# mit-acl/clipper

Measured on AMD Instinct MI355X. Metric: affinity+solve ms and GEMV HBM GB/s, n=10k assoc, 95% outliers, 1/8 GPU, lower is better.
Workload: dtype f64 (M stored f32)

## Files before the change

### clipper_amd/csrc/host_solver.hpp

```cpp
#pragma once

namespace {

using Ctx = clipper_hip_ctx;

void rowview_free(Shard& s);
void rowview_drop(Ctx* h);
void sub_free(Ctx* h);

int free_shard_buffers(Shard& s) {
  hipSetDevice(s.device);
  auto fr = [](auto*& p) {
    if (p) hipFree(p);
    p = nullptr;
  };
  fr(s.S);
  fr(s.Cs);
  fr(s.part);
  fr(s.u0);
  fr(s.pt);
  fr(s.cab);
  fr(s.X[0]);
  fr(s.X[1]);
  fr(s.ab);
// ... 83 lines not shown
  for (auto& s : h->sh) {
    free_shard_buffers(s);
    HIPCHK(hipSetDevice(s.device));
    const size_t bytesS = static_cast<size_t>(m) * static_cast<size_t>(W) * h->esize();
    s.bytes_S = bytesS;
    if (!h->compressed) HIPCHK(hipMalloc(&s.S, bytesS));
    const size_t nvec = static_cast<size_t>(P * W) * sizeof(double);
    const size_t V = static_cast<size_t>(h->V);
    HIPCHK(hipMalloc(&s.u0, nvec));
    const size_t NSLOT = static_cast<size_t>(nslot(h->V));
    HIPCHK(hipMalloc(&s.pt, 2 * V * 2 * nvec));
    HIPCHK(hipMalloc(&s.cab, 2 * nvec));
    for (int k = 0; k < 2; ++k) {
      HIPCHK(hipMalloc(&s.X[k], (V + 1) * VS * nvec));
      HIPCHK(hipMemsetAsync(s.X[k], 0, (V + 1) * VS * nvec, s.stream));
    }
    const size_t Q = static_cast<size_t>(tail_q(h->V));
    const size_t nwg = static_cast<size_t>(ceil_div(m, TAIL_THREADS));
    HIPCHK(hipMalloc(&s.scal, (nwg + ceil_div(nwg, SCAL_FOLD) + 1) * Q * sizeof(double)));
    HIPCHK(hipMalloc(&s.ab, NSLOT * nvec));
    HIPCHK(hipMemsetAsync(s.ab, 0, NSLOT * nvec, s.stream));
    s.part_tiles = static_cast<size_t>(max_tiles(h));
    HIPCHK(hipMalloc(&s.part, s.part_tiles * NSLOT * W * sizeof(double)));
    HIPCHK(hipMalloc(&s.st, 2 * sizeof(SolverState)));
    HIPCHK(hipMemsetAsync(s.st, 0, 2 * sizeof(SolverState), s.stream));
    HIPCHK(hipMalloc(&s.shared, sizeof(SolveShared)));
    HIPCHK(hipMalloc(&s.marks, KIND_CAP));
    HIPCHK(hipMemsetAsync(s.marks, 0, KIND_CAP, s.stream));
    HIPCHK(hipMemsetAsync(s.shared, 0, sizeof(SolveShared), s.stream));
  }
  h->alloc_m = m;
  h->alloc_W = W;
  h->has_matrix = false;
  h->csc_valid = false;
  h->explicitC = false;
  plan_tiles(h);
  h->u0_staged = false;
  h->staged_d = 0;
  return 0;
}

template <typename T, bool HASC, int V>
void launch_pass_tv(Ctx* h, Shard& s, const SolveArgs& a) {
  constexpr int UNR = gemv_unr(V, sizeof(T), HASC);
  dim3 grid(h->nstrips, h->ntiles), block(GEMV_NW * 64);
  hipLaunchKernelGGL((k_gemv<T, HASC, V, GEMV_NW, UNR>), grid, block, 0, s.stream,
                     static_cast<const T*>(s.S), static_cast<const T*>(s.Cs), h->rows_per_tile, a);
}
// ... 120 lines not shown
  for (auto& q : h->sh) {
    HIPCHK(hipSetDevice(q.device));
    for (auto& p : h->sh) {
      if (p.slot == q.slot) continue;
      HIPCHK(hipStreamWaitEvent(q.stream, p.ev_reduced, 0));
      const int64_t off = static_cast<int64_t>(p.slot) * blk_elems;
      if (p.device == q.device) {
        HIPCHK(hipMemcpyAsync(q.ab + off, p.ab + off, blk, hipMemcpyDeviceToDevice, q.stream));
      } else {
        HIPCHK(hipMemcpyPeerAsync(q.ab + off, q.device, p.ab + off, p.device, blk, q.stream));
      }
    }
    HIPCHK(hipEventRecord(q.ev_copied, q.stream));
  }
  for (auto& p : h->sh) {
    HIPCHK(hipSetDevice(p.device));
    for (auto& q : h->sh) {
      if (p.slot == q.slot) continue;
      HIPCHK(hipStreamWaitEvent(p.stream, q.ev_copied, 0));
    }
  }
  return 0;
}

SolveArgs solve_args(Ctx* h, Shard& s, const SolverParams& prm, int par, bool decide_only) {
  SolveArgs a;
  a.st_cur = s.st + par;
  a.st_next = s.st + (par ^ 1);
  a.shared = s.shared;
  a.host = (&s == &h->sh[0]) ? h->mirror_dev : nullptr;
  a.prm = prm;
  a.m = h->m;
  a.W = h->W;
  a.mp = h->mp;
  a.u0 = s.u0;
  a.pt = s.pt;
  a.cab = s.cab;
  a.Xin = s.X[par];
  a.Xout = s.X[par ^ 1];
  a.ab = s.ab;
  a.part = s.part;
  a.ntiles = h->csc_valid ? s.s_nslots : h->ntiles;
  a.slot = s.slot;
  a.scal = s.scal;
  a.nwg = static_cast<int>(ceil_div(h->m, TAIL_THREADS));
  a.scal_in = s.scal;
// ... 16 lines not shown
  a.rvp = h->rvp;
  a.decide_only = decide_only ? 1 : 0;
  a.adaptive_window = (h->csc_valid && h->world == 1 && !h->multiproc && h->sh.size() == 1 && h->adaptive_window) ? 1 : 0;
  a.sub_state = 0;
  a.sub_ncol = 0.0;
  a.colmap = nullptr;
  if (h->parent != nullptr) {
    Ctx* p = h->parent;
    a.host = p->mirror_dev;
    a.host_u = p->u_pinned_dev;
    a.marks = p->profiling ? p->sh[0].marks : nullptr;
    a.kind = a.marks ? p->kind_dev : nullptr;
    a.stamps = p->stamps_dev;
    a.stamps_wide = p->stamps_rows > 4096 ? 1 : 0;
    a.sub_state = 2;
    a.sub_ncol = p->sub.ncol;
    a.colmap = p->sub.colmap;
    static const int test_leave = std::getenv("CLIPPER_HIP_SUB_TEST_LEAVE") ? std::atoi(std::getenv("CLIPPER_HIP_SUB_TEST_LEAVE")) : 0;
    if (test_leave > 0 && p->sub.launches_since_entry >= test_leave) a.sub_ncol = 1e300;
  } else if (h->sub.ready && !h->sub.active && !decide_only) {
    a.sub_state = 1;
    a.sub_ncol = h->sub.ncol;
  }
  return a;
}

template <int V>
int enqueue_iteration_v(Ctx* h, const SolverParams& prm, bool decide_only) {
  const int par = h->par;
  h->par ^= 1;
  const bool sharded = !(h->world == 1 && !h->multiproc);
  Shard& s0 = h->sh[0];
  constexpr int every = PROFILE_EVERY;
  Ctx* hp = h->parent != nullptr ? h->parent : h;
  const bool prof = hp->profiling && (hp->launch_counter % every == 4 || hp->launch_counter == 11) &&
                    hp->ev_used < MAX_EVENT_PAIRS;
  for (auto& s : h->sh) {
    HIPCHK(hipSetDevice(s.device));
    const SolveArgs a = solve_args(h, s, prm, par, decide_only);
    if (prof && &s == &s0) HIPCHK(hipEventRecord(hp->ev_pairs[2 * hp->ev_used], s.stream));
    if (h->csc_valid) launch_pass_csc<V>(h, s, a);
    else launch_pass<V>(h, s, a);
    if (prof && &s == &s0) {
      HIPCHK(hipEventRecord(hp->ev_pairs[2 * hp->ev_used + 1], s.stream));
      hp->ev_launch_index[hp->ev_used] = hp->launch_counter;
      ++hp->ev_used;
// ... 177 lines not shown
    return nullptr;
  }
  std::memset(h->mirror, 0, sizeof(HostMirror));
  if (hipHostMalloc(reinterpret_cast<void**>(&h->kind), KIND_CAP,
                    hipHostMallocMapped | hipHostMallocCoherent) != hipSuccess ||
      hipHostGetDevicePointer(reinterpret_cast<void**>(&h->kind_dev), h->kind, 0) != hipSuccess) {
    fail(CLIPPER_HIP_E_HIP, "cannot allocate the pinned iteration marks");
    destroy_ctx(h);
    return nullptr;
  }
  std::memset(h->kind, 0, KIND_CAP);
  if (const char* e = std::getenv("CLIPPER_HIP_STAMPS")) {
    h->stamps_rows = std::atoi(e) == 2 ? 16384 : 4096;
    const size_t bytes = static_cast<size_t>(h->stamps_rows) * 4 * sizeof(long long);
    if (hipMalloc(&h->stamps_dev, bytes) == hipSuccess) (void)hipMemset(h->stamps_dev, 0, bytes);
    else h->stamps_dev = nullptr;
  }
  if (const char* w = std::getenv("CLIPPER_HIP_WINDOW")) {
    const int v = std::atoi(w);
    if (v == 1 || v == 4 || v == 6 || v == 8) h->V_forced = v;
  }
  if (const char* e = std::getenv("CLIPPER_HIP_ADAPTIVE_WINDOW"))
    if (std::atoi(e) == 0) h->adaptive_window = false;
  if (const char* e = std::getenv("CLIPPER_HIP_RESIDENT"))
    if (std::atoi(e) == 0) h->resident_mode = 1;
  return h;
}

template <typename T>
int ensure_cap(T*& p, size_t& cap, size_t bytes) {
  if (bytes <= cap && p) return 0;
  if (p) hipFree(p);
  p = nullptr;
  cap = 0;
  HIPCHK(hipMalloc(&p, bytes));
  cap = bytes;
  return 0;
}

int upload_points(Ctx* h, Shard& s, const double* D1, const double* D2, int d, int64_t n1,
                  int64_t n2, int64_t pstride, const StagedInputs* dev = nullptr) {
  const size_t b1 = static_cast<size_t>(d) * n1 * sizeof(double);
  const size_t b2 = static_cast<size_t>(d) * n2 * sizeof(double);
  const size_t bp = static_cast<size_t>(d) * pstride * sizeof(double);
  const size_t ba = static_cast<size_t>(2 * h->m) * sizeof(int32_t);
  int rc;
// ... 126 lines not shown
```

### clipper_amd/csrc/host_state.hpp

```cpp
#pragma once

namespace {

thread_local std::string g_err;

int fail(int code, const char* fmt, ...) {
  char buf[512];
  va_list ap;
  va_start(ap, fmt);
  vsnprintf(buf, sizeof(buf), fmt, ap);
  va_end(ap);
  g_err = buf;
  return code;
}

int guard_fail(int code, const char* what) noexcept {
  try {
    g_err = what;
  } catch (...) {
  }
  return code;
}
#define CLIPPER_HIP_GUARD_CATCH(on_nomem, on_other)                                                     \
  catch (const std::bad_alloc&) { on_nomem; }                                                            \
// ... 289 lines not shown
  const SolverParams* solve_prm = nullptr;
  bool early_decide_done = false;
  int resident_mode = 0;
  bool borrowed_stream = false;
  int last_solver = 0;

  int fill_kind = 0;
  EuclidParams fill_e{};
  PointNormalParams fill_n{};
  float fill_E2 = 0.f;
  double total_slice_bytes = 0.0;
  ViewPolicy rvp{};
  bool rv_fresh = false;
  int rv_mode = 0;
  SliceView* rv_desc_host = nullptr;
  int rv_desc_slot = 0;
  SliceView* rv_desc_host_dev = nullptr;
  int32_t* rv_count = nullptr;
  int32_t* rv_count_dev = nullptr;
  clipper_hip_view_stats_t rv_stats{};
  SubProblem sub;
  struct clipper_hip_ctx* parent = nullptr;
  bool adaptive_window = true;
  int sub_mode = 0;

  long long* stamps_dev = nullptr;
  int stamps_rows = 4096;
  bool profiling = false;
  int profiling_level = 0;
  std::vector<hipEvent_t> ev_pairs;
  std::vector<int64_t> ev_launch_index;
  std::vector<hipEvent_t> ev_xchg;
  std::vector<char> ev_xchg_used;
  int ev_used = 0;
  int64_t launch_counter = 0;
  clipper_hip_timings_t tm{};

  size_t esize() const { return storage == CLIPPER_HIP_STORE_F64 ? 8 : 4; }
};
```

### clipper_amd/csrc/host_subproblem.hpp

```cpp
#pragma once

namespace {

bool sub_enabled(const Ctx* h) {
  static const bool env_off = [] {
    const char* e = std::getenv("CLIPPER_HIP_SUBPROBLEM");
    return e && std::atoi(e) == 0;
  }();
  static const int64_t min_m = std::getenv("CLIPPER_HIP_SUBPROBLEM_MIN_M") ? std::atoll(std::getenv("CLIPPER_HIP_SUBPROBLEM_MIN_M")) : SUB_MIN_M;
  return !env_off && h->sub_mode != 1 && h->parent == nullptr && h->sh.size() == 1 && h->world == 1 && !h->multiproc &&
         h->csc_valid && !h->explicitC && h->m >= min_m && rect_fill_possible(h);
}

void sub_begin_solve(Ctx* h) {
  SubProblem& sp = h->sub;
  sp.ready = sp.active = false;
  sp.entries = 0;
  sp.sub_passes = sp.leaves = 0;
  sp.build_ms = 0.0;
}

void sub_free(Ctx* h) {
  SubProblem& sp = h->sub;
  for (Ctx** pc : {&sp.ctx, &sp.ctx_dense}) {
// ... 149 lines not shown
                 (c->csc_valid ? static_cast<double>(c->sh[0].s_bytes) : algorithmic_gemv_bytes(c)) * 1e-6, sp.build_ms);
  return 0;
}

int sub_prepare(Ctx* h) {
  int rc = 0;
  dispatch_window(h, [&](auto v) { rc = sub_prepare_v<decltype(v)::value>(h); });
  return rc;
}

int sub_enter(Ctx* h, const SolverParams& prm) {
  SubProblem& sp = h->sub;
  if (!sp.ready || sp.active || !sp.use) return fail(CLIPPER_HIP_E_INTERNAL, "sub-problem: a hand-over nobody prepared");
  Shard& s = h->sh[0];
  Ctx* c = sp.use;
  Shard& cs = c->sh[0];
  HIPCHK(hipSetDevice(s.device));
  hipLaunchKernelGGL(k_sub_resume, dim3(1), dim3(64), 0, s.stream, s.st + h->par, s.shared);
  if (int rc = enqueue_iteration(h, prm, true)) return rc;
  std::memset(h->u_pinned, 0, static_cast<size_t>(h->m) * sizeof(double));
  std::atomic_thread_fence(std::memory_order_seq_cst);
  hipLaunchKernelGGL(k_sub_enter, dim3(static_cast<unsigned>(ceil_div(c->mp, 256))), dim3(256), 0, s.stream, s.st + h->par, s.pt,
                     s.cab, h->mp, h->V, sp.colmap, sp.nS, cs.st, cs.shared, cs.pt, cs.cab, c->mp,
                     c->csc_valid ? static_cast<double*>(nullptr) : cs.X[0], prm.beta);
  c->par = 0;
  c->rv_fresh = false;
  sp.active = true;
  sp.entries += 1;
  sp.launches_since_entry = 0;
  sp.passes_at_entry = h->mirror->n_passes;
  h->rv_stats.sub_entries += 1;
  return 0;
}

int sub_leave(Ctx* h) {
  SubProblem& sp = h->sub;
  if (!sp.active || !sp.use) return fail(CLIPPER_HIP_E_INTERNAL, "sub-problem: nothing to leave");
  Shard& s = h->sh[0];
  Ctx* c = sp.use;
  Shard& cs = c->sh[0];
  HIPCHK(hipSetDevice(s.device));
  hipLaunchKernelGGL(k_sub_leave, dim3(static_cast<unsigned>(ceil_div(h->mp, 256))), dim3(256), 0, s.stream, cs.st + c->par, cs.pt,
                     cs.cab, c->mp, h->V, sp.pos, s.rv.in_view[s.rv.cur], h->m, s.pt, s.cab, h->mp, sp.nout_acc);
  hipLaunchKernelGGL(k_sub_leave_state, dim3(1), dim3(256), 0, s.stream, cs.st + c->par, s.st + h->par, s.shared, sp.nout_acc);
  sp.active = false;
  sp.leaves += 1;
  if (sp.entries >= SUB_MAX_ENTRIES) sp.ready = false;
// ... 5 lines not shown
```

### clipper_amd/csrc/k_solver.hip.h

```cpp
#pragma once

#include <hip/hip_runtime.h>
#include <stdint.h>
#include <type_traits>


namespace clipper_hip {


constexpr int VS = 8;
constexpr int nslot(int V) { return V + 1; }
constexpr int tail_nr(int V) { return 3 + 2 * V; }
constexpr int tail_q(int V) { return V * tail_nr(V) + 2 * V + 2; }

constexpr double LIVE_OUT = 67108864.0;
constexpr double RV_GAIN_MARGIN = 1.3;
constexpr double RV_ROWS_RATIO = 0.8;

struct ViewPolicy {
  int32_t on;
  int32_t max_builds;
  double pass_fixed, pass_per_row;
  double build_fixed, build_per_row;
};
// ... 21 lines not shown
  double sx[VS];
  int32_t sel;
  int32_t ubp, ubv;
  int32_t phase;
  int32_t stage;
  int32_t i, j, k;
  int64_t n_passes;
  int64_t n_trials;
  int64_t n_iters;
  int32_t nlive;
  int32_t nout;
  int32_t view;
  int32_t hold;
  int64_t n_view_passes;
  int32_t rv_builds;
  int32_t rv_last;
  int32_t rv_backoff;
  int32_t hold_slot;
  int32_t hold_nlive;
  int32_t resume;
  int32_t weff;
  int32_t zero_run;
  int32_t n_redo;
  int32_t pad_;
};

struct SolveShared {
  double F, d;
  int64_t n_passes, n_trials;
  int32_t ifinal, ubp, ubv;
  int32_t done;
  int32_t hold;
  int32_t pad;
};

struct HostMirror {
  double F, d;
  int64_t n_passes, n_trials;
  int64_t iters;
  int32_t ifinal, ubp, ubv;
  int32_t done;
  int32_t nlive, nout;
  int64_t n_view_passes;
  int32_t hold;
  int32_t hold_nlive;
};

// ... 4 lines not shown
  double tol_u, tol_F, beta, eps;
  int32_t maxiniters, maxoliters, maxlsiters;
};


__device__ __forceinline__ double cl_project(double u, double al, double g) {
  const double t = u + al * g;
  return (t > 0.0) ? t : 0.0;
}

__device__ __forceinline__ double cl_norm(double z, bool use = true) { return (use && z > 0.0) ? sqrt(z) : 1.0; }

__device__ __forceinline__ double cl_grad(double d, double x, double s, double a, double b) {
  return (1 + d) * x - d * s + a + b * d;
}
__device__ __forceinline__ double cl_grad_fused(double d, double x, double s, double gs) {
  return (1 + d) * x - d * s + gs;
}

__device__ __forceinline__ double cl_pen_cbu(double s, double b, double u) { return s - b - u; }
__device__ __forceinline__ bool cl_pen_in(double cbu, double u, double eps) { return cbu > eps && u > eps; }
__device__ __forceinline__ double cl_pen_ratio(double a, double u, double cbu) { return fabs((a + u) / cbu); }
__device__ __forceinline__ double cl_pen_ratio_init(double a, double u, double cbu) { return (a + u) / cbu; }

constexpr double SUB_ENTER_MARGIN = 1.10;
constexpr double SUB_STAY_MARGIN = 1.01;

constexpr int TAIL_THREADS = 256;
constexpr int TAIL_WAVES = TAIL_THREADS / 64;
constexpr int TAIL_SPLIT = 1;

struct SolveArgs {
  const SolverState* st_cur;
  SolverState* st_next;
  SolveShared* shared;
  HostMirror* host;
  SolverParams prm;
  int64_t m;
  int64_t W;
  int64_t mp;
  const double* u0;
  double* pt;
  double* cab;
  const double* Xin;
  double* Xout;
  double* ab;
  double* part;
  int ntiles;
  int slot;
  double* scal;
  int nwg;
  const double* scal_in;
  int nwg_in;
  uint8_t* marks;
  uint8_t* kind;
  double* host_u;
  long long* stamps;
  int stamps_wide;
  const uint8_t* in_view;
  int rv_nslots;
  int rv_nwork;
  int rv_fresh;
  int rv_rows;
  ViewPolicy rvp;
  int decide_only;
  int adaptive_window;
  int sub_state;
  double sub_ncol;
  const int32_t* colmap;
};
constexpr int KIND_CAP = 1 << 16;


__device__ __forceinline__ double* pt_arr(const SolveArgs& A, int V, int p, int v, int k) {
  return A.pt + ((static_cast<int64_t>(p) * V + v) * 2 + k) * A.mp;
}

template <int CTRL, int ROW_MASK>
__device__ __forceinline__ double dpp_f64(double v) {
  const int lo = __builtin_amdgcn_update_dpp(0, __double2loint(v), CTRL, ROW_MASK, 0xf, false);
  const int hi = __builtin_amdgcn_update_dpp(0, __double2hiint(v), CTRL, ROW_MASK, 0xf, false);
  return __hiloint2double(hi, lo);
}

__device__ __forceinline__ double wave_sum_to_lane63(double v) {
  v += dpp_f64<0xB1, 0xf>(v);
  v += dpp_f64<0x4E, 0xf>(v);
  v += dpp_f64<0x141, 0xf>(v);
  v += dpp_f64<0x140, 0xf>(v);
  v += dpp_f64<0x142, 0xa>(v);
  v += dpp_f64<0x143, 0xc>(v);
  return v;
// ... 196 lines not shown
  int i_ = L.i, j_ = L.j, k_ = L.k, ubp = L.ubp, ubv = L.ubv, sel = L.sel;
  const int wprev = (L.weff >= 1 && L.weff <= V) ? L.weff : V;
  int zero_run = L.zero_run;
  int64_t n_passes = L.n_passes, n_trials = L.n_trials;
  const int64_t n_iters = L.n_iters + 1;
  int nlive = L.nlive, nout = L.nout;
  auto live_code = [&](double code) {
    const double o = floor(code * (1.0 / LIVE_OUT));
    nout = static_cast<int>(o);
    nlive = static_cast<int>(code - o * LIVE_OUT);
  };
  if (writer && tid == 0) {
#pragma unroll
    for (int l = 0; l < V; ++l) {
      stash->nrm[l] = 1.0;
      stash->sx[l] = 0.0;
    }
  }
  enum { ACT_PASS, ACT_BUILD, ACT_SLOW, ACT_DONE };
  int action = ACT_SLOW;
  int next_phase = PH_TRIAL;
  bool need_pair = false;
  bool redo = false;
  bool sub_ok = true;
  auto sub_bound = [&](const double* sums, int nb) {
    if (A.sub_state == 0) return;
    const double kap = (A.sub_state == 1 ? SUB_ENTER_MARGIN : SUB_STAY_MARGIN) * A.sub_ncol;
    const double lhs = d * d, rhs = (1.0 + d) * (1.0 + d) * kap;
#pragma unroll
    for (int l = 0; l < V; ++l) {
      const double z = sums[nb + 2 * l], sl = sums[nb + 2 * l + 1];
      sub_ok = sub_ok && (lhs * sl * sl >= rhs * z);
    }
  };

  if (phase == PH_TRIAL || phase == PH_BUILD) {
    {
      red[tid] = L.chain;
      __syncthreads();
      double tot = 0.0;
      if (tid < QPAD) {
        tot = red[tid];
#pragma unroll
        for (int c2 = 1; c2 < NCH; ++c2) tot += red[c2 * QPAD + tid];
      }
      __syncthreads();
// ... 103 lines not shown
      } else {
        alpha = 1.0;
        k_ = 0;
        sel = 0;
        action = ACT_PASS;
        sub_bound(sums, 2);
        if (writer && tid == 0) {
#pragma unroll
          for (int l = 0; l < V; ++l) {
            const double nl = cl_norm(sums[2 + 2 * l]);
            stash->nrm[l] = nl;
            stash->sx[l] = sums[3 + 2 * l] / nl;
          }
        }
      }
    }
  }

  if (action == ACT_SLOW) {
    if (!writer) return false;
    nlive = nout = static_cast<int>(m < 0x7fffffff ? m : 0x7fffffff);
    const double* ca_ = A.cab;
    const double* cb_ = A.cab + A.mp;
    if (phase == PH_NORMALIZE || phase == PH_RESCALE) {
      double* u = pt_arr(A, V, ubp, ubv, 0);
      double z[1] = {0.0};
      VEC_CHUNKS(base) {
        double uv[VU], av[VU];
        VEC_EACH(k, i, base) {
          uv[k] = A.u0[i];
          if (phase == PH_RESCALE) av[k] = ca_[i];
        }
        VEC_EACH(k, i, base) {
          const double ui = (phase == PH_RESCALE) ? av[k] + uv[k] : uv[k];
          u[i] = ui;
          z[0] += ui * ui;
        }
      }
      block_reduce<1, NWV>(z, scratch);
      const double n0 = sqrt(z[0]);
      VEC_CHUNKS(base) {
        double uv[VU];
        VEC_EACH(k, i, base) uv[k] = u[i];
        VEC_EACH(k, i, base) {
          const double ui = uv[k] / n0;
          u[i] = ui;
          const double row[VS] = {ui, 0.0, 0.0, 0.0, 0.0, 0.0, 0.0, 0.0};
          store_row(A.Xout + i * VS, row);
        }
      }
      sel = 0;
      next_phase = PH_INIT;
    } else {
      if (phase == PH_INIT) {
        const double* u = pt_arr(A, V, ubp, ubv, 0);
        double sv[1] = {0.0};
        VEC_CHUNKS(base) {
          double uv[VU];
          VEC_EACH(k, i, base) uv[k] = u[i];
          VEC_EACH(k, i, base) sv[0] += uv[k];
        }
        block_reduce<1, NWV>(sv, scratch);
        s = sv[0];
        double ca[2] = {0.0, 0.0};
        VEC_CHUNKS(base) {
          double uv[VU], av[VU], bv[VU];
          VEC_EACH(k, i, base) {
            uv[k] = u[i];
            av[k] = ca_[i];
            bv[k] = cb_[i];
          }
          VEC_EACH(k, i, base) {
            const double cbu = cl_pen_cbu(s, bv[k], uv[k]);
            if (cl_pen_in(cbu, uv[k], P.eps)) {
              ca[0] += 1.0;
              ca[1] += cl_pen_ratio_init(av[k], uv[k], cbu);
            }
          }
        }
        block_reduce<2, NWV>(ca, scratch);
        d = (ca[0] > 0.0) ? ca[1] / ca[0] : 0.0;
        i_ = 0;
        action = (i_ >= P.maxoliters) ? ACT_DONE : ACT_BUILD;
      } else {
        const double* u = pt_arr(A, V, ubp, ubv, 0);
        double ca[2] = {0.0, 0.0};
        VEC_CHUNKS(base) {
          double uv[VU], av[VU], bv[VU];
          VEC_EACH(k, i, base) {
            uv[k] = u[i];
            av[k] = ca_[i];
            bv[k] = cb_[i];
          }
          VEC_EACH(k, i, base) {
            const double cbu = cl_pen_cbu(s, bv[k], uv[k]);
            if (cl_pen_in(cbu, uv[k], P.eps)) {
              ca[0] += 1.0;
              ca[1] += cl_pen_ratio(av[k], uv[k], cbu);
            }
          }
        }
        block_reduce<2, NWV>(ca, scratch);
        if (ca[0] > 0.0) {
          d += ca[1] / ca[0];
          ++i_;
          action = (i_ >= P.maxoliters) ? ACT_DONE : ACT_BUILD;
        } else {
          action = ACT_DONE;
        }
      }
    }
  }

  if (writer && action == ACT_DONE && A.host_u != nullptr) {
    const double* u = pt_arr(A, V, ubp, ubv, 0);
    for (int64_t i = tid; i < m; i += NT)
      __hip_atomic_store(A.host_u + (A.colmap != nullptr ? static_cast<int64_t>(A.colmap[i]) : i), u[i], __ATOMIC_RELAXED,
                         __HIP_MEMORY_SCOPE_SYSTEM);
    if (A.kind != nullptr && A.marks != nullptr) {
      const int64_t n = (n_iters < KIND_CAP) ? n_iters : KIND_CAP;
      for (int64_t i = tid; i < n; i += NT)
        __hip_atomic_store(A.kind + i, A.marks[i], __ATOMIC_RELAXED, __HIP_MEMORY_SCOPE_SYSTEM);
    }
    __threadfence_system();
    __syncthreads();
  }

  if (A.rv_fresh != 0 && action != ACT_SLOW) nout = 0;
  auto put_on_hold = [&](int reason) {
    if (writer) {
      copy_state(A.st_next, st, tid, NT);
      __syncthreads();
// ... 40 lines not shown
      o->ubv = ubv;
      o->phase = (action == ACT_BUILD) ? static_cast<int>(PH_BUILD) : next_phase;
      o->stage = (action == ACT_SLOW) ? ST_PASS : ST_RESULTS;
      o->i = i_;
      o->j = j_;
      o->k = k_;
      o->n_passes = n_passes + (action == ACT_PASS ? 1 : 0);
      o->n_trials = n_trials;
      o->n_iters = n_iters;
      o->nlive = nlive;
      o->nout = nout;
      o->view = (action == ACT_PASS && on_view) ? 1 : 0;
      o->hold = 0;
      o->n_view_passes = L.n_view_passes + ((action == ACT_PASS && on_view) ? 1 : 0);
      o->rv_builds = L.rv_builds;
      o->rv_last = L.rv_last;
      o->rv_backoff = L.rv_backoff;
      o->hold_slot = 0;
      o->hold_nlive = 0;
      o->resume = 0;
      o->weff = wnext;
      o->zero_run = zero_run;
      o->n_redo = L.n_redo + (redo ? 1 : 0);
      o->pad_ = 0;
    };
    if (action == ACT_PASS) record(stash, true);
    else record(A.st_next, false);
    if ((A.decide_only != 0 || sub_leave) && action == ACT_PASS) {
      stash->stage = ST_PASS;
      stash->resume = need_pair ? 2 : 1;
      stash->n_passes = n_passes;
      stash->view = 0;
      stash->n_view_passes = L.n_view_passes;
      if (sub_leave) {
        stash->hold = HOLD_SUB_LEAVE;
        A.shared->hold = HOLD_SUB_LEAVE;
      }
    }
    if (action == ACT_DONE) {
      SolveShared* sh = A.shared;
      sh->F = F;
      sh->d = d;
      sh->n_passes = n_passes;
      sh->n_trials = n_trials;
      sh->ifinal = i_;
      sh->ubp = ubp;
      sh->ubv = ubv;
// ... 92 lines not shown
            al = al * beta;
          }
        }
      }
      block_reduce<2 * V, NT / 64>(r, lds);
      if (threadIdx.x == 0) {
#pragma unroll
        for (int l = 0; l < V; ++l) {
          const double z = (all_rows ? 0.0 : stash->nrm[l]) + r[2 * l], sm = (all_rows ? 0.0 : stash->sx[l]) + r[2 * l + 1];
          const double nl = cl_norm(z);
          stash->nrm[l] = nl;
          stash->sx[l] = sm / nl;
        }
      }
      __syncthreads();
    }
    if (threadIdx.x == 0) {
      stash->stage = ST_RESULTS;
      stash->n_passes = L.n_passes + 1;
      stash->n_iters = L.n_iters + 1;
      stash->view = on_view;
      stash->n_view_passes = L.n_view_passes + on_view;
      stash->resume = 0;
      stash->weff = plan.weff;
    }
  }
  return true;
}

__device__ __forceinline__ void flush_state(const SolveArgs& A, const SolverState* stash) {
  if (!is_writer_block()) return;
  copy_state(A.st_next, stash, threadIdx.x, blockDim.x);
  if (threadIdx.x == 0) {
    const int64_t n_iters = stash->n_iters;
    if (A.marks != nullptr && n_iters <= KIND_CAP)
      A.marks[n_iters - 1] = A.sub_state == 2 ? (stash->phase == PH_TRIAL ? MARK_SUB_WINDOW : MARK_SUB_PAIR)
                             : stash->view   ? MARK_VIEW
                                             : (stash->phase == PH_TRIAL ? MARK_WINDOW : MARK_PAIR);
    if (A.host != nullptr) {
      __hip_atomic_store(&A.host->nlive, stash->nlive, __ATOMIC_RELAXED, __HIP_MEMORY_SCOPE_SYSTEM);
      __hip_atomic_store(&A.host->nout, stash->nout, __ATOMIC_RELAXED, __HIP_MEMORY_SCOPE_SYSTEM);
      __hip_atomic_store(&A.host->n_view_passes, stash->n_view_passes, __ATOMIC_RELAXED, __HIP_MEMORY_SCOPE_SYSTEM);
      __hip_atomic_store(&A.host->n_passes, stash->n_passes, __ATOMIC_RELAXED, __HIP_MEMORY_SCOPE_SYSTEM);
      __hip_atomic_store(&A.host->iters, n_iters, __ATOMIC_RELEASE, __HIP_MEMORY_SCOPE_SYSTEM);
    }
  }
}

__global__ __launch_bounds__(256) void k_init(SolveArgs A, SolverState init, SolverState* st0,
                                               double* X0) {
  const int64_t i = static_cast<int64_t>(blockIdx.x) * 256 + threadIdx.x;
  if (i < A.m) {
    const double row[VS] = {A.u0[i], 0.0, 0.0, 0.0, 0.0, 0.0, 0.0, 0.0};
    store_row(X0 + i * VS, row);
  }
  if (blockIdx.x == 0) {
    if (threadIdx.x == 0) {
      *st0 = init;
      A.shared->done = 0;
      A.shared->hold = 0;
    }
  }
}

constexpr int SCAL_FOLD = 32;
constexpr int SCAL_FOLD_MIN = 64;
__global__ __launch_bounds__(128) void k_scal_fold(const double* __restrict__ scal, int nwg, int Q,
                                                    double* __restrict__ out,
                                                    const SolveShared* __restrict__ shared) {
  if (shared->done) return;
  const int w0 = blockIdx.x * SCAL_FOLD;
  const int w1 = (w0 + SCAL_FOLD < nwg) ? w0 + SCAL_FOLD : nwg;
  for (int q = threadIdx.x; q < Q; q += 128) {
    double x[SCAL_FOLD];
#pragma unroll
    for (int k = 0; k < SCAL_FOLD; ++k) {
      const int w = (w0 + k < w1) ? w0 + k : w1 - 1;
      x[k] = scal[static_cast<int64_t>(w) * Q + q];
    }
    double acc = 0.0;
#pragma unroll
    for (int k = 0; k < SCAL_FOLD; ++k)
      if (w0 + k < w1) acc += x[k];
    out[static_cast<int64_t>(blockIdx.x) * Q + q] = acc;
  }
}

template <int V, bool FUSED_REDUCE, bool TABLES = true>
__global__ __launch_bounds__(TAIL_THREADS * (FUSED_REDUCE ? TAIL_SPLIT : 1)) void k_tail(SolveArgs A) {
  constexpr int NR = tail_nr(V);
  constexpr int Q = tail_q(V);
  constexpr int NRED = NR + 2 * V + 2;
  constexpr int NSLOT = nslot(V);
  constexpr int NTW = TAIL_WAVES * (FUSED_REDUCE ? TAIL_SPLIT : 1);
  __shared__ double red[NTW * NRED > 2 * TAIL_SPLIT * TAIL_THREADS ? NTW * NRED : 2 * TAIL_SPLIT * TAIL_THREADS];
  const int v = blockIdx.y;
  const long long c0 = A.stamps ? wall_clock64() : 0;
  const SolverState* st = A.st_next;
  const int te = threadIdx.x & (TAIL_THREADS - 1);
  const int grp = threadIdx.x / TAIL_THREADS;
  const int64_t i = static_cast<int64_t>(blockIdx.x) * TAIL_THREADS + te;
  const bool valid = i < A.m && grp == 0;
  const int done = A.shared->done;
  const int stage = st->stage, phase = st->phase;
  const int ubp = st->ubp, ubv = st->ubv, sel = st->sel;
  const double d = st->d, alpha = st->alpha, s_cur = st->s;
  const double nrmv = st->nrm[v], sxv = st->sx[v];
  const int weff = (st->weff >= 1 && st->weff <= V) ? st->weff : V;
  const int nslots_pass = st->view ? A.rv_nslots : A.ntiles;
  const double live_w = (valid && A.in_view != nullptr && A.in_view[i] == 0) ? 1.0 + LIVE_OUT : 1.0;

  double p0 = 0.0, p1 = 0.0;
  if (FUSED_REDUCE) {
    const int64_t o1 = (v == 0) ? static_cast<int64_t>(V) * A.W : 0;
    const int per = (nslots_pass + TAIL_SPLIT - 1) / TAIL_SPLIT;
    const int t0 = grp * per, t1 = (t0 + per < nslots_pass) ? t0 + per : nslots_pass;
    if (i < A.m) {
      const double* p = A.part + static_cast<int64_t>(v) * A.W + i;
      const int64_t ts = static_cast<int64_t>(NSLOT) * A.W;
      for (int t = t0; t < t1; t += 16) {
        double va[16], vb[16];
#pragma unroll
        for (int q = 0; q < 16; ++q) {
          const int tt = (t + q < t1) ? t + q : t1 - 1;
          va[q] = p[static_cast<int64_t>(tt) * ts];
          vb[q] = p[static_cast<int64_t>(tt) * ts + o1];
        }
#pragma unroll
        for (int q = 0; q < 16; ++q) {
          if (t + q < t1) {
// ... 6 lines not shown
    if constexpr (TAIL_SPLIT > 1) {
      red[(grp * 2 + 0) * TAIL_THREADS + te] = p0;
      red[(grp * 2 + 1) * TAIL_THREADS + te] = p1;
      __syncthreads();
      p0 = red[te];
      p1 = red[TAIL_THREADS + te];
#pragma unroll
      for (int g = 1; g < TAIL_SPLIT; ++g) {
        p0 += red[(g * 2 + 0) * TAIL_THREADS + te];
        p1 += red[(g * 2 + 1) * TAIL_THREADS + te];
      }
      __syncthreads();
    }
  } else if (valid) {
    const int64_t o1 = (v == 0) ? static_cast<int64_t>(V) * A.W : 0;
    const uint32_t pb = static_cast<uint32_t>(i) / static_cast<uint32_t>(A.W);
    const int64_t off = i - static_cast<int64_t>(pb) * A.W;
    const double* blk = A.ab + (static_cast<int64_t>(pb) * NSLOT) * A.W;
    p0 = blk[static_cast<int64_t>(v) * A.W + off];
    p1 = blk[o1 + off];
  }
  if (done) return;
  if (st->hold) return;
  if (stage != ST_RESULTS) return;
  if (phase == PH_TRIAL && v >= weff) return;
  const long long c1 = A.stamps ? wall_clock64() + (p0 > 1e300 ? 1 : 0) : 0;

  if (phase != PH_TRIAL && phase != PH_BUILD) {
    if (v == 0 && valid) {
      A.cab[i] = p0;
      A.cab[A.mp + i] = p1;
    }
    return;
  }
  const double beta = A.prm.beta;
  double r[NRED];
#pragma unroll
  for (int q = 0; q < NRED; ++q) r[q] = 0.0;

  if (phase == PH_BUILD) {
    if (v != 0) return;
    if (valid) {
      const double ui = pt_arr(A, V, ubp, ubv, 0)[i];
      const double gi = (1 + d) * ui - d * s_cur + A.cab[i] + A.cab[A.mp + i] * d;
      pt_arr(A, V, ubp, ubv, 1)[i] = gi;
      r[0] = ui * gi;
      r[NR - 1] = (ui > 0.0 || gi > 0.0) ? live_w : 0.0;
      double row[VS] = {0.0, 0.0, 0.0, 0.0, 0.0, 0.0, 0.0, 0.0};
      double al = 1.0;
#pragma unroll
      for (int l = 0; l < V; ++l) {
        const double t = cl_project(ui, al, gi);
        row[l] = t;
        r[2 + 2 * l] = t * t;
        r[3 + 2 * l] = t;
// ... 84 lines not shown
```

### clipper_amd/csrc/k_subproblem.hip.h

```cpp
#pragma once

#include <hip/hip_runtime.h>
#include <stdint.h>

#include "k_rowview.hip.h"
#include "k_slices.hip.h"
#include "k_solver.hip.h"

namespace clipper_hip {

constexpr double SUB_THETA = 0.4;

__global__ __launch_bounds__(256) void k_sub_colcount(SliceView RV, int32_t* __restrict__ cnt, int64_t mp) {
  const int lane = threadIdx.x & 63;
  const int cg = blockIdx.x * 4 + (threadIdx.x >> 6);
  if (cg >= RV.ncg) return;
  const uint64_t* pre = RV.Pre + static_cast<int64_t>(cg) * RV.nchunks;
  int tot = 0;
  for (int k0 = 0; k0 < RV.nchunks; k0 += 8) {
    uint8_t nq[8];
#pragma unroll
    for (int j = 0; j < 8; ++j) {
      const int k = (k0 + j < RV.nchunks) ? k0 + j : RV.nchunks - 1;
      nq[j] = RV.data[16 * pre[k] + 16 + lane];
// ... 77 lines not shown
}

__global__ __launch_bounds__(256) void k_sub_gather_points(const double* __restrict__ P, const float* __restrict__ Pf,
                                                            int d, int64_t pstride, const int32_t* __restrict__ A,
                                                            int64_t m, const int32_t* __restrict__ colmap, int64_t nS,
                                                            int64_t qstride, double* __restrict__ Q,
                                                            float* __restrict__ Qf, int32_t* __restrict__ B,
                                                            int which) {
  const int64_t i = static_cast<int64_t>(blockIdx.x) * 256 + threadIdx.x;
  if (i >= qstride) return;
  const int64_t c = (i < nS) ? colmap[i] : 0;
  for (int k = 0; k < d; ++k) {
    Q[k * qstride + i] = (i < nS) ? P[k * pstride + c] : 0.0;
    Qf[k * qstride + i] = (i < nS) ? Pf[k * pstride + c] : 0.f;
  }
  if (i < nS) B[which * nS + i] = A[which * m + c];
}

__global__ __launch_bounds__(256) void k_sub_enter(const SolverState* __restrict__ pst, const double* __restrict__ ppt,
                                                    const double* __restrict__ pcab, int64_t pmp, int V,
                                                    const int32_t* __restrict__ colmap, int64_t nS,
                                                    SolverState* __restrict__ cst, SolveShared* __restrict__ cshared,
                                                    double* __restrict__ cpt, double* __restrict__ ccab, int64_t cmp,
                                                    double* __restrict__ ctab, double beta) {
  const int64_t i = static_cast<int64_t>(blockIdx.x) * 256 + threadIdx.x;
  const int64_t slot = static_cast<int64_t>(pst->ubp) * V + pst->ubv;
  if (i < cmp) {
    const bool in = i < nS;
    const int64_t c = in ? colmap[i] : 0;
    const double ui = in ? ppt[(slot * 2 + 0) * pmp + c] : 0.0;
    const double gi = in ? ppt[(slot * 2 + 1) * pmp + c] : 0.0;
    cpt[(slot * 2 + 0) * cmp + i] = ui;
    cpt[(slot * 2 + 1) * cmp + i] = gi;
    ccab[i] = in ? pcab[c] : 0.0;
    ccab[cmp + i] = in ? pcab[pmp + c] : 0.0;
    if (ctab != nullptr && pst->resume == 1) {
      double row[VS] = {0.0, 0.0, 0.0, 0.0, 0.0, 0.0, 0.0, 0.0};
      double al = pst->alpha;
      for (int l = 0; l < V; ++l) {
        row[l] = cl_project(ui, al, gi);
        al = al * beta;
      }
      store_row(ctab + (static_cast<int64_t>(pst->sel) * cmp + i) * VS, row);
    }
  }
  if (blockIdx.x == 0) {
    copy_state(cst, pst, threadIdx.x, 256);
    __syncthreads();
    if (threadIdx.x == 0) {
      cst->hold = 0;
      cst->nout = 0;
      cst->view = 0;
      cshared->done = 0;
      cshared->hold = 0;
    }
  }
}

__global__ __launch_bounds__(256) void k_sub_leave(const SolverState* __restrict__ cst, const double* __restrict__ cpt,
                                                    const double* __restrict__ ccab, int64_t cmp, int V,
                                                    const int32_t* __restrict__ pos, const uint8_t* __restrict__ in_view,
                                                    int64_t m, double* __restrict__ ppt, double* __restrict__ pcab,
                                                    int64_t pmp, int32_t* __restrict__ nout_acc) {
  const int64_t c = static_cast<int64_t>(blockIdx.x) * 256 + threadIdx.x;
  const int64_t slot = static_cast<int64_t>(cst->ubp) * V + cst->ubv;
  int out = 0;
  if (c < pmp) {
    const int64_t i = (c < m) ? pos[c] : -1;
    double u = 0.0, g = (c < m) ? -1.0 : 0.0, a = 0.0, b = 0.0;
    if (i >= 0) {
      u = cpt[(slot * 2 + 0) * cmp + i];
      g = cpt[(slot * 2 + 1) * cmp + i];
      a = ccab[i];
      b = ccab[cmp + i];
      out = ((u > 0.0 || g > 0.0) && in_view[c] == 0) ? 1 : 0;
    }
    ppt[(slot * 2 + 0) * pmp + c] = u;
// ... 29 lines not shown
```

Before: 1.300.

## Move phase-transition reductions into a last-block tail sweep of the pass kernel

The reductions the single-block decide step used to run at phase transitions (the norm for normalize/rescale, the sum and penalty counts for init/outlier updates) now run once at the end of the preceding pass. The last workgroup to finish, chosen with an atomic ticket, does the sweep with a wider thread count and records the results in a SweepRecord that the decide step reuses when iteration and phase match. The normalization write-back of u and Xout moves into the next pass kernel, driven by the new tnorm and n0 state fields. This is meant to cut serial single-block sweeps over m from the decide kernel's critical path. In exchange the pass kernel gains an atomic handoff, extra fences and a serial tail executed by one workgroup.

```diff
diff --git a/clipper_amd/csrc/host_solver.hpp b/clipper_amd/csrc/host_solver.hpp
--- a/clipper_amd/csrc/host_solver.hpp
+++ b/clipper_amd/csrc/host_solver.hpp
@@ -129,8 +129,8 @@
     HIPCHK(hipMemsetAsync(s.ab, 0, NSLOT * nvec, s.stream));
     s.part_tiles = static_cast<size_t>(max_tiles(h));
     HIPCHK(hipMalloc(&s.part, s.part_tiles * NSLOT * W * sizeof(double)));
-    HIPCHK(hipMalloc(&s.st, 2 * sizeof(SolverState)));
-    HIPCHK(hipMemsetAsync(s.st, 0, 2 * sizeof(SolverState), s.stream));
+    HIPCHK(hipMalloc(&s.st, 2 * sizeof(SolverState) + sizeof(SweepRecord)));
+    HIPCHK(hipMemsetAsync(s.st, 0, 2 * sizeof(SolverState) + sizeof(SweepRecord), s.stream));
     HIPCHK(hipMalloc(&s.shared, sizeof(SolveShared)));
     HIPCHK(hipMalloc(&s.marks, KIND_CAP));
     HIPCHK(hipMemsetAsync(s.marks, 0, KIND_CAP, s.stream));
@@ -297,6 +297,8 @@
   }
   return 0;
 }
+
+inline SweepRecord* sweep_record(const Shard& s) { return reinterpret_cast<SweepRecord*>(s.st + 2); }
 
 SolveArgs solve_args(Ctx* h, Shard& s, const SolverParams& prm, int par, bool decide_only) {
   SolveArgs a;
@@ -359,6 +361,9 @@
     a.sub_state = 1;
     a.sub_ncol = h->sub.ncol;
   }
+  a.rec = sweep_record(s);
+  a.tail_sweeps = (h->parent != nullptr ? h->parent->tail_sweeps : h->tail_sweeps) ? 1 : 0;
+  a.NT = (h->csc_valid ? SL_NW : GEMV_NW) * 64;
   return a;
 }
 
@@ -582,6 +587,8 @@
   }
   if (const char* e = std::getenv("CLIPPER_HIP_ADAPTIVE_WINDOW"))
     if (std::atoi(e) == 0) h->adaptive_window = false;
+  if (const char* e = std::getenv("CLIPPER_HIP_TAIL_SWEEPS"))
+    if (std::atoi(e) == 0) h->tail_sweeps = false;
   if (const char* e = std::getenv("CLIPPER_HIP_RESIDENT"))
     if (std::atoi(e) == 0) h->resident_mode = 1;
   return h;
diff --git a/clipper_amd/csrc/host_state.hpp b/clipper_amd/csrc/host_state.hpp
--- a/clipper_amd/csrc/host_state.hpp
+++ b/clipper_amd/csrc/host_state.hpp
@@ -335,6 +335,7 @@
   SubProblem sub;
   struct clipper_hip_ctx* parent = nullptr;
   bool adaptive_window = true;
+  bool tail_sweeps = true;
   int sub_mode = 0;
 
   long long* stamps_dev = nullptr;
diff --git a/clipper_amd/csrc/host_subproblem.hpp b/clipper_amd/csrc/host_subproblem.hpp
--- a/clipper_amd/csrc/host_subproblem.hpp
+++ b/clipper_amd/csrc/host_subproblem.hpp
@@ -195,7 +195,7 @@
   std::atomic_thread_fence(std::memory_order_seq_cst);
   hipLaunchKernelGGL(k_sub_enter, dim3(static_cast<unsigned>(ceil_div(c->mp, 256))), dim3(256), 0, s.stream, s.st + h->par, s.pt,
                      s.cab, h->mp, h->V, sp.colmap, sp.nS, cs.st, cs.shared, cs.pt, cs.cab, c->mp,
-                     c->csc_valid ? static_cast<double*>(nullptr) : cs.X[0], prm.beta);
+                     c->csc_valid ? static_cast<double*>(nullptr) : cs.X[0], prm.beta, sweep_record(cs));
   c->par = 0;
   c->rv_fresh = false;
   sp.active = true;
diff --git a/clipper_amd/csrc/k_solver.hip.h b/clipper_amd/csrc/k_solver.hip.h
--- a/clipper_amd/csrc/k_solver.hip.h
+++ b/clipper_amd/csrc/k_solver.hip.h
@@ -67,7 +67,17 @@
   int32_t weff;
   int32_t zero_run;
   int32_t n_redo;
-  int32_t pad_;
+  int32_t tnorm;
+  double n0;
+};
+
+struct SweepRecord {
+  double z;
+  double s;
+  double cnt, ratio;
+  int64_t n_iters;
+  int32_t phase;
+  uint32_t ticket;
 };
 
 struct SolveShared {
@@ -118,6 +128,18 @@
 __device__ __forceinline__ bool cl_pen_in(double cbu, double u, double eps) { return cbu > eps && u > eps; }
 __device__ __forceinline__ double cl_pen_ratio(double a, double u, double cbu) { return fabs((a + u) / cbu); }
 __device__ __forceinline__ double cl_pen_ratio_init(double a, double u, double cbu) { return (a + u) / cbu; }
+
+__device__ __forceinline__ double cl_sw_u(bool rescale, double a, double u0) { return rescale ? a + u0 : u0; }
+__device__ __forceinline__ void cl_sw_sq(double& z, double ui) { z += ui * ui; }
+__device__ __forceinline__ void cl_sw_sum(double& s, double u) { s += u; }
+__device__ __forceinline__ void cl_sw_pen(double& cnt, double& ratio, double s, double u, double a, double b, double eps,
+                                          bool init) {
+  const double cbu = cl_pen_cbu(s, b, u);
+  if (cl_pen_in(cbu, u, eps)) {
+    cnt += 1.0;
+    ratio += init ? cl_pen_ratio_init(a, u, cbu) : cl_pen_ratio(a, u, cbu);
+  }
+}
 
 constexpr double SUB_ENTER_MARGIN = 1.10;
 constexpr double SUB_STAY_MARGIN = 1.01;
@@ -164,6 +186,9 @@
   int sub_state;
   double sub_ncol;
   const int32_t* colmap;
+  SweepRecord* rec;
+  int tail_sweeps;
+  int NT;
 };
 constexpr int KIND_CAP = 1 << 16;
 
@@ -406,6 +431,8 @@
   int next_phase = PH_TRIAL;
   bool need_pair = false;
   bool redo = false;
+  int tnorm = 0;
+  double n0 = 0.0;
   bool sub_ok = true;
   auto sub_bound = [&](const double* sums, int nb) {
     if (A.sub_state == 0) return;
@@ -555,47 +582,69 @@
     nlive = nout = static_cast<int>(m < 0x7fffffff ? m : 0x7fffffff);
     const double* ca_ = A.cab;
     const double* cb_ = A.cab + A.mp;
+    const bool tsw = A.tail_sweeps != 0;
+    const SweepRecord* rec = A.rec;
+    const int64_t rec_iters = rec->n_iters;
+    const int rec_phase = rec->phase;
+    const double rec_z = rec->z, rec_s = rec->s, rec_cnt = rec->cnt, rec_ratio = rec->ratio;
+    const bool rec_ok = tsw && rec_iters == L.n_iters && rec_phase == phase;
     if (phase == PH_NORMALIZE || phase == PH_RESCALE) {
+      const bool rescale = phase == PH_RESCALE;
       double* u = pt_arr(A, V, ubp, ubv, 0);
       double z[1] = {0.0};
-      VEC_CHUNKS(base) {
-        double uv[VU], av[VU];
-        VEC_EACH(k, i, base) {
-          uv[k] = A.u0[i];
-          if (phase == PH_RESCALE) av[k] = ca_[i];
-        }
-        VEC_EACH(k, i, base) {
-          const double ui = (phase == PH_RESCALE) ? av[k] + uv[k] : uv[k];
-          u[i] = ui;
-          z[0] += ui * ui;
-        }
-      }
-      block_reduce<1, NWV>(z, scratch);
-      const double n0 = sqrt(z[0]);
-      VEC_CHUNKS(base) {
-        double uv[VU];
-        VEC_EACH(k, i, base) uv[k] = u[i];
-        VEC_EACH(k, i, base) {
-          const double ui = uv[k] / n0;
-          u[i] = ui;
-          const double row[VS] = {ui, 0.0, 0.0, 0.0, 0.0, 0.0, 0.0, 0.0};
-          store_row(A.Xout + i * VS, row);
+      if (rec_ok) {
+        z[0] = rec_z;
+      } else {
+        VEC_CHUNKS(base) {
+          double uv[VU], av[VU] = {0.0, 0.0, 0.0, 0.0};
+          VEC_EACH(k, i, base) {
+            uv[k] = A.u0[i];
+            if (rescale) av[k] = ca_[i];
+          }
+          VEC_EACH(k, i, base) {
+            const double ui = cl_sw_u(rescale, av[k], uv[k]);
+            if (!tsw) u[i] = ui;
+            cl_sw_sq(z[0], ui);
+          }
+        }
+        block_reduce<1, NWV>(z, scratch);
+      }
+      n0 = sqrt(z[0]);
+      if (tsw) {
+        tnorm = rescale ? 2 : 1;
+      } else {
+        VEC_CHUNKS(base) {
+          double uv[VU];
+          VEC_EACH(k, i, base) uv[k] = u[i];
+          VEC_EACH(k, i, base) {
+            const double ui = uv[k] / n0;
+            u[i] = ui;
+            const double row[VS] = {ui, 0.0, 0.0, 0.0, 0.0, 0.0, 0.0, 0.0};
+            store_row(A.Xout + i * VS, row);
+          }
         }
       }
       sel = 0;
       next_phase = PH_INIT;
     } else {
-      if (phase == PH_INIT) {
+      const bool init = phase == PH_INIT;
+      double ca[2] = {0.0, 0.0};
+      if (rec_ok) {
+        if (init) s = rec_s;
+        ca[0] = rec_cnt;
+        ca[1] = rec_ratio;
+      } else {
         const double* u = pt_arr(A, V, ubp, ubv, 0);
-        double sv[1] = {0.0};
-        VEC_CHUNKS(base) {
-          double uv[VU];
-          VEC_EACH(k, i, base) uv[k] = u[i];
-          VEC_EACH(k, i, base) sv[0] += uv[k];
-        }
-        block_reduce<1, NWV>(sv, scratch);
-        s = sv[0];
-        double ca[2] = {0.0, 0.0};
+        if (init) {
+          double sv[1] = {0.0};
+          VEC_CHUNKS(base) {
+            double uv[VU];
+            VEC_EACH(k, i, base) uv[k] = u[i];
+            VEC_EACH(k, i, base) cl_sw_sum(sv[0], uv[k]);
+          }
+          block_reduce<1, NWV>(sv, scratch);
+          s = sv[0];
+        }
         VEC_CHUNKS(base) {
           double uv[VU], av[VU], bv[VU];
           VEC_EACH(k, i, base) {
@@ -603,44 +652,20 @@
             av[k] = ca_[i];
             bv[k] = cb_[i];
           }
-          VEC_EACH(k, i, base) {
-            const double cbu = cl_pen_cbu(s, bv[k], uv[k]);
-            if (cl_pen_in(cbu, uv[k], P.eps)) {
-              ca[0] += 1.0;
-              ca[1] += cl_pen_ratio_init(av[k], uv[k], cbu);
-            }
-          }
+          VEC_EACH(k, i, base) cl_sw_pen(ca[0], ca[1], s, uv[k], av[k], bv[k], P.eps, init);
         }
         block_reduce<2, NWV>(ca, scratch);
+      }
+      if (init) {
         d = (ca[0] > 0.0) ? ca[1] / ca[0] : 0.0;
         i_ = 0;
         action = (i_ >= P.maxoliters) ? ACT_DONE : ACT_BUILD;
+      } else if (ca[0] > 0.0) {
+        d += ca[1] / ca[0];
+        ++i_;
+        action = (i_ >= P.maxoliters) ? ACT_DONE : ACT_BUILD;
       } else {
-        const double* u = pt_arr(A, V, ubp, ubv, 0);
-        double ca[2] = {0.0, 0.0};
-        VEC_CHUNKS(base) {
-          double uv[VU], av[VU], bv[VU];
-          VEC_EACH(k, i, base) {
-            uv[k] = u[i];
-            av[k] = ca_[i];
-            bv[k] = cb_[i];
-          }
-          VEC_EACH(k, i, base) {
-            const double cbu = cl_pen_cbu(s, bv[k], uv[k]);
-            if (cl_pen_in(cbu, uv[k], P.eps)) {
-              ca[0] += 1.0;
-              ca[1] += cl_pen_ratio(av[k], uv[k], cbu);
-            }
-          }
-        }
-        block_reduce<2, NWV>(ca, scratch);
-        if (ca[0] > 0.0) {
-          d += ca[1] / ca[0];
-          ++i_;
-          action = (i_ >= P.maxoliters) ? ACT_DONE : ACT_BUILD;
-        } else {
-          action = ACT_DONE;
-        }
+        action = ACT_DONE;
       }
     }
   }
@@ -727,7 +752,8 @@
       o->weff = wnext;
       o->zero_run = zero_run;
       o->n_redo = L.n_redo + (redo ? 1 : 0);
-      o->pad_ = 0;
+      o->tnorm = tnorm;
+      o->n0 = n0;
     };
     if (action == ACT_PASS) record(stash, true);
     else record(A.st_next, false);
@@ -866,6 +892,7 @@
       stash->view = on_view;
       stash->n_view_passes = L.n_view_passes + on_view;
       stash->resume = 0;
+      stash->tnorm = 0;
       stash->weff = plan.weff;
     }
   }
@@ -903,6 +930,9 @@
       *st0 = init;
       A.shared->done = 0;
       A.shared->hold = 0;
+      A.rec->n_iters = -1;
+      A.rec->phase = -1;
+      A.rec->ticket = 0u;
     }
   }
 }
@@ -927,6 +957,112 @@
     for (int k = 0; k < SCAL_FOLD; ++k)
       if (w0 + k < w1) acc += x[k];
     out[static_cast<int64_t>(blockIdx.x) * Q + q] = acc;
+  }
+}
+
+constexpr int SW_LOADS = 24;
+constexpr int SW_MAX_NT = 1024;
+
+template <int NQ, int NA, typename Term>
+__device__ __forceinline__ void tail_sweep(const double* const (&arr)[NA], int64_t m, int NT, double (&tot)[NQ],
+                                           double* lds , Term term) {
+  constexpr int SW_U = SW_LOADS / NA < 16 ? SW_LOADS / NA : 16;
+  const int t = threadIdx.x;
+  for (int c = t; c < NT; c += TAIL_THREADS) {
+    double acc[NQ];
+#pragma unroll
+    for (int q = 0; q < NQ; ++q) acc[q] = 0.0;
+    for (int64_t i0 = c; i0 < m; i0 += static_cast<int64_t>(NT) * SW_U) {
+      double x[SW_U][NA];
+#pragma unroll
+      for (int e = 0; e < SW_U; ++e) {
+        const int64_t i = i0 + static_cast<int64_t>(e) * NT;
+        const int64_t ii = (i < m) ? i : i0;
+#pragma unroll
+        for (int a = 0; a < NA; ++a) x[e][a] = arr[a][ii];
+      }
+#pragma unroll
+      for (int e = 0; e < SW_U; ++e)
+        if (i0 + static_cast<int64_t>(e) * NT < m) term(acc, x[e]);
+    }
+#pragma unroll
+    for (int q = 0; q < NQ; ++q) acc[q] = wave_sum_to_lane63(acc[q]);
+    if ((t & 63) == 63) {
+#pragma unroll
+      for (int q = 0; q < NQ; ++q) lds[(c >> 6) * NQ + q] = acc[q];
+    }
+  }
+  __syncthreads();
+  const int nwv = NT >> 6;
+#pragma unroll
+  for (int q = 0; q < NQ; ++q) {
+    double acc = lds[q];
+    for (int w = 1; w < nwv; ++w) acc += lds[w * NQ + q];
+    tot[q] = acc;
+  }
+  __syncthreads();
+}
+
+template <int V>
+__device__ __forceinline__ void tail_transition_sums(const SolveArgs& A, int phase, int ubp, int ubv, double s_cur,
+                                                     int64_t n_iters, double* lds) {
+  static_assert(TAIL_SPLIT == 1, "the workgroup's TAIL_THREADS threads sweep");
+  SweepRecord* rec = A.rec;
+  asm volatile("s_waitcnt vmcnt(0)" ::: "memory");
+  __syncthreads();
+  if (threadIdx.x == 0) {
+    __builtin_amdgcn_fence(__ATOMIC_RELEASE, "agent");
+    asm volatile("s_waitcnt vmcnt(0)" ::: "memory");
+    const unsigned tk = __hip_atomic_fetch_add(&rec->ticket, 1u, __ATOMIC_RELAXED, __HIP_MEMORY_SCOPE_AGENT);
+    const bool mine = tk == gridDim.x - 1u;
+    if (mine) {
+      __builtin_amdgcn_fence(__ATOMIC_ACQUIRE, "agent");
+      asm volatile("s_waitcnt vmcnt(0)" ::: "memory");
+    }
+    lds[0] = mine ? 1.0 : 0.0;
+  }
+  __syncthreads();
+  const bool last = lds[0] != 0.0;
+  __syncthreads();
+  if (!last) return;
+
+  const int64_t m = A.m;
+  const int NT = A.NT;
+  const double eps = A.prm.eps;
+  const double* ca_ = A.cab;
+  const double* cb_ = A.cab + A.mp;
+  double z = 0.0, s = s_cur, cnt = 0.0, ratio = 0.0;
+  if (phase == PH_RESCALE) {
+    const double* const arr[2] = {A.u0, ca_};
+    double tot[1];
+    tail_sweep<1, 2>(arr, m, NT, tot, lds,
+                     [](double (&acc)[1], const double (&x)[2]) { cl_sw_sq(acc[0], cl_sw_u(true, x[1], x[0])); });
+    z = tot[0];
+  } else {
+    const bool init = phase == PH_INIT;
+    const double* u = pt_arr(A, V, ubp, ubv, 0);
+    if (init) {
+      const double* const arr[1] = {u};
+      double tot[1];
+      tail_sweep<1, 1>(arr, m, NT, tot, lds, [](double (&acc)[1], const double (&x)[1]) { cl_sw_sum(acc[0], x[0]); });
+      s = tot[0];
+    }
+    const double* const arr[3] = {u, ca_, cb_};
+    double tot[2];
+    tail_sweep<2, 3>(arr, m, NT, tot, lds, [=](double (&acc)[2], const double (&x)[3]) {
+      cl_sw_pen(acc[0], acc[1], s, x[0], x[1], x[2], eps, init);
+    });
+    cnt = tot[0];
+    ratio = tot[1];
+  }
+  if (threadIdx.x == 0) {
+    rec->z = z;
+    rec->s = s;
+    rec->cnt = cnt;
+    rec->ratio = ratio;
+    rec->n_iters = n_iters;
+    rec->phase = phase;
+    __hip_atomic_store(&rec->ticket, 0u, __ATOMIC_RELAXED, __HIP_MEMORY_SCOPE_AGENT);
   }
 }
 
@@ -950,6 +1086,9 @@
   const int ubp = st->ubp, ubv = st->ubv, sel = st->sel;
   const double d = st->d, alpha = st->alpha, s_cur = st->s;
   const double nrmv = st->nrm[v], sxv = st->sx[v];
+  const int tnorm = st->tnorm;
+  const double n0 = st->n0;
+  const int64_t st_iters = st->n_iters;
   const int weff = (st->weff >= 1 && st->weff <= V) ? st->weff : V;
   const int nslots_pass = st->view ? A.rv_nslots : A.ntiles;
   const double live_w = (valid && A.in_view != nullptr && A.in_view[i] == 0) ? 1.0 + LIVE_OUT : 1.0;
@@ -1002,7 +1141,16 @@
   }
   if (done) return;
   if (st->hold) return;
-  if (stage != ST_RESULTS) return;
+  if (stage != ST_RESULTS) {
+    if (tnorm != 0 && v == 0 && valid) {
+      const double a = (tnorm == 2) ? A.cab[i] : 0.0;
+      const double ui = cl_sw_u(tnorm == 2, a, A.u0[i]) / n0;
+      pt_arr(A, V, ubp, ubv, 0)[i] = ui;
+      const double row[VS] = {ui, 0.0, 0.0, 0.0, 0.0, 0.0, 0.0, 0.0};
+      store_row(A.Xout + i * VS, row);
+    }
+    return;
+  }
   if (phase == PH_TRIAL && v >= weff) return;
   const long long c1 = A.stamps ? wall_clock64() + (p0 > 1e300 ? 1 : 0) : 0;
 
@@ -1011,6 +1159,8 @@
       A.cab[i] = p0;
       A.cab[A.mp + i] = p1;
     }
+    if (v == 0 && A.tail_sweeps != 0 && phase != PH_NORMALIZE)
+      tail_transition_sums<V>(A, phase, ubp, ubv, s_cur, st_iters, red);
     return;
   }
   const double beta = A.prm.beta;
diff --git a/clipper_amd/csrc/k_subproblem.hip.h b/clipper_amd/csrc/k_subproblem.hip.h
--- a/clipper_amd/csrc/k_subproblem.hip.h
+++ b/clipper_amd/csrc/k_subproblem.hip.h
@@ -123,7 +123,7 @@
                                                     const int32_t* __restrict__ colmap, int64_t nS,
                                                     SolverState* __restrict__ cst, SolveShared* __restrict__ cshared,
                                                     double* __restrict__ cpt, double* __restrict__ ccab, int64_t cmp,
-                                                    double* __restrict__ ctab, double beta) {
+                                                    double* __restrict__ ctab, double beta, SweepRecord* __restrict__ crec) {
   const int64_t i = static_cast<int64_t>(blockIdx.x) * 256 + threadIdx.x;
   const int64_t slot = static_cast<int64_t>(pst->ubp) * V + pst->ubv;
   if (i < cmp) {
@@ -154,6 +154,9 @@
       cst->view = 0;
       cshared->done = 0;
       cshared->hold = 0;
+      crec->n_iters = -1;
+      crec->phase = -1;
+      crec->ticket = 0u;
     }
   }
 }
```

New measurement: 1.288 (median of 6 runs). About the same (-0.9%).
